# openai/gym

Measured on AMD Instinct MI355X. Metric: env-steps/sec at num_envs=2^20, CartPole-v1, higher is better.
Workload: dtype f64

## Files before the change

gym_amd/csrc/mxv_subnorm.hip:

```cpp
#include <hip/hip_runtime.h>

#include <cmath>
#include <cstdint>
#include <new>
#include <string>
#include <vector>

#include "../../include/mxv.h"
#include "mxv_divide.hpp"
#include "mxv_host.hpp"

using mxv::check_aligned;
using mxv::fail;
using mxv::last_error;

namespace {

constexpr int kThreads = 256;

template <int D>
__device__ __forceinline__ void load_row(const float *base, int64_t row, float (&v)[D]) {
    if constexpr (D == 4) {
        const float4 q = reinterpret_cast<const float4 *>(base)[row];
        v[0] = q.x; v[1] = q.y; v[2] = q.z; v[3] = q.w;
    } else if constexpr (D == 2) {
        const float2 q = reinterpret_cast<const float2 *>(base)[row];
        v[0] = q.x; v[1] = q.y;
    } else if constexpr (D == 6) {
        const float2 *p = reinterpret_cast<const float2 *>(base) + row * 3;
        const float2 a = p[0], b = p[1], c = p[2];
        v[0] = a.x; v[1] = a.y; v[2] = b.x; v[3] = b.y; v[4] = c.x; v[5] = c.y;
    } else {
#pragma unroll
        for (int j = 0; j < D; ++j) v[j] = base[row * D + j];
    }
}

template <int D>
__device__ __forceinline__ void store_row(float *base, int64_t row, const double (&y)[D]) {
    if constexpr (D == 4) {
        reinterpret_cast<float4 *>(base)[row] = make_float4((float)y[0], (float)y[1], (float)y[2], (float)y[3]);
    } else if constexpr (D == 2) {
        reinterpret_cast<float2 *>(base)[row] = make_float2((float)y[0], (float)y[1]);
    } else if constexpr (D == 6) {
        float2 *p = reinterpret_cast<float2 *>(base) + row * 3;
        p[0] = make_float2((float)y[0], (float)y[1]);
        p[1] = make_float2((float)y[2], (float)y[3]);
        p[2] = make_float2((float)y[4], (float)y[5]);
    } else {
#pragma unroll
        for (int j = 0; j < D; ++j) base[row * D + j] = (float)y[j];
    }
}

template <int D>
__device__ __forceinline__ void store_row(double *base, int64_t row, const double (&y)[D]) {
    if constexpr (D % 2 == 0) {
        double2 *p = reinterpret_cast<double2 *>(base) + row * (D / 2);
#pragma unroll
        for (int j = 0; j < D / 2; ++j) p[j] = make_double2(y[2 * j], y[2 * j + 1]);
    } else {
#pragma unroll
        for (int j = 0; j < D; ++j) base[row * D + j] = y[j];
    }
}

using mxv::div_shared;
using mxv::plain_delta;
using mxv::plain_divisor;
using mxv::plain_operand;
using mxv::refined_rcp;

template <int D>
__device__ __forceinline__ void update_one(const float (&x)[D], double (&mean)[D], double (&var)[D], double &count) {
    const double tot = count + 1.0;
    double delta[D], sq[D];
    bool ok = plain_divisor(tot) && (plain_divisor(count) || count == 0.0);
#pragma unroll
    for (int j = 0; j < D; ++j) {
        delta[j] = (double)x[j] - mean[j];
        sq[j] = (delta[j] * delta[j]) * count;
        ok = ok && plain_delta(delta[j]);
    }
    if (__all(ok)) {
        const double r = refined_rcp(tot);
        double m2[D];
        bool ok2 = true;
#pragma unroll
        for (int j = 0; j < D; ++j) {
            m2[j] = var[j] * count + div_shared(sq[j], tot, r);
            mean[j] = mean[j] + div_shared(delta[j], tot, r);
            ok2 = ok2 && plain_operand(m2[j]);
        }
        if (__all(ok2)) {
#pragma unroll
            for (int j = 0; j < D; ++j) var[j] = div_shared(m2[j], tot, r);
        } else {
#pragma unroll
            for (int j = 0; j < D; ++j) var[j] = m2[j] / tot;
        }
    } else {
#pragma unroll
        for (int j = 0; j < D; ++j) {
            const double m2 = var[j] * count + sq[j] / tot;
            mean[j] = mean[j] + delta[j] / tot;
            var[j] = m2 / tot;
        }
    }
    count = tot;
}

template <int D>
__device__ __forceinline__ void normalise(const float (&x)[D], const double (&mean)[D], const double (&var)[D], double eps, double (&y)[D]) {
#pragma unroll
    for (int j = 0; j < D; ++j) y[j] = ((double)x[j] - mean[j]) / sqrt(var[j] + eps);
}

struct SubObsArgs {
    const float *x;
    const float *fin;
    const uint8_t *te, *tr;
    void *y;
    double *yfin;
    double *stat;
    int64_t n;
    int32_t K;
    double eps;
};

template <int D, typename OUT>
__global__ void __launch_bounds__(kThreads) subnorm_obs_kernel(const SubObsArgs a) {
    const int64_t e = (int64_t)blockIdx.x * kThreads + threadIdx.x;
    const bool mine = e < a.n;
    const int64_t ec = mine ? e : 0;
    double mean[D], var[D], count;
#pragma unroll
    for (int j = 0; j < D; ++j) {
        mean[j] = a.stat[(int64_t)j * a.n + ec];
        var[j] = a.stat[(int64_t)(D + j) * a.n + ec];
    }
    count = a.stat[(int64_t)(2 * D) * a.n + ec];
    int kl = mine ? 0 : a.K;
    bool fin_done = false;
    const bool has_fin = a.te != nullptr && a.fin != nullptr;
    while (__any(kl < a.K)) {
        if (kl < a.K) {
            const int64_t r = (int64_t)kl * a.n + e;
            const bool use_fin = has_fin && !fin_done && ((a.te[r] | a.tr[r]) != 0);
            float x[D];
            load_row<D>(use_fin ? a.fin : a.x, r, x);
            double y[D];
            update_one<D>(x, mean, var, count);
            normalise<D>(x, mean, var, a.eps, y);
            if (use_fin) {
                if (a.yfin != nullptr) store_row<D>(a.yfin, r, y);
                fin_done = true;
            } else {
                store_row<D>(static_cast<OUT *>(a.y), r, y);
                fin_done = false;
                kl += 1;
            }
        }
    }
    if (!mine) return;
#pragma unroll
    for (int j = 0; j < D; ++j) {
        a.stat[(int64_t)j * a.n + e] = mean[j];
        a.stat[(int64_t)(D + j) * a.n + e] = var[j];
    }
    a.stat[(int64_t)(2 * D) * a.n + e] = count;
}

struct SubRewArgs {
    const void *rew;
    const uint8_t *te, *tr;
    void *out;
    double *stat;
    double *returns;
    int64_t n;
    int32_t K;
    double gamma, eps;
};

template <typename RT>
__global__ void __launch_bounds__(kThreads) subnorm_rew_kernel(const SubRewArgs a) {
    const int64_t e = (int64_t)blockIdx.x * kThreads + threadIdx.x;
    if (e >= a.n) return;
    double mean = a.stat[e], var = a.stat[a.n + e], count = a.stat[2 * a.n + e], ret = a.returns[e];
    const RT *rew = static_cast<const RT *>(a.rew);
    RT *out = static_cast<RT *>(a.out);
    for (int k = 0; k < a.K; ++k) {
        const int64_t r = (int64_t)k * a.n + e;
        const double rw = (double)rew[r];
        const bool done = (a.te[r] | a.tr[r]) != 0;
        ret = ret * a.gamma + rw;
        {
            const double tot = count + 1.0, delta = ret - mean, sq = (delta * delta) * count;
            const bool ok = plain_divisor(tot) && (plain_divisor(count) || count == 0.0) && plain_delta(delta);
            if (__all(ok)) {
                const double rc = refined_rcp(tot);
                const double m2 = var * count + div_shared(sq, tot, rc);
                mean = mean + div_shared(delta, tot, rc);
                var = __all(plain_operand(m2)) ? div_shared(m2, tot, rc) : m2 / tot;
            } else {
                const double m2 = var * count + sq / tot;
                mean = mean + delta / tot;
                var = m2 / tot;
            }
            count = tot;
        }
        out[r] = (RT)(rw / sqrt(var + a.eps));
        if (done) ret = 0.0;
    }
    a.stat[e] = mean;
    a.stat[a.n + e] = var;
    a.stat[2 * a.n + e] = count;
    a.returns[e] = ret;
}

}

struct mxv_subnorm {
    static constexpr const char *kNullMessage = "NULL mxv_subnorm";
    int device = 0, dim = 0;
    int64_t n = 0;
    hipStream_t stream = nullptr;
    double *stat = nullptr;
    double *returns = nullptr;
    std::string error;
};

namespace {

bool sub_dim_supported(int d) { return d == 1 || d == 2 || d == 3 || d == 4 || d == 6; }

int sub_checks(mxv_subnorm *nm, int32_t K) {
    MXV_CHECK(nm);
    if (K <= 0) return fail(nm, MXV_ERR_INVALID_ARG, "K must be positive (got %d)", K);
    if ((int64_t)K * nm->n > ((int64_t)1 << 40)) return fail(nm, MXV_ERR_INVALID_ARG, "K * num_envs too large");
    MXV_HIP(nm, hipSetDevice(nm->device));
    return MXV_OK;
}

int init_stats(mxv_subnorm *nm) {
    const size_t n = (size_t)nm->n;
    std::vector<double> init((size_t)(2 * nm->dim + 1) * n, 0.0);
    for (size_t i = (size_t)nm->dim * n; i < (size_t)(2 * nm->dim) * n; ++i) init[i] = 1.0;
    for (size_t i = (size_t)(2 * nm->dim) * n; i < init.size(); ++i) init[i] = 1e-4;
    MXV_HIP(nm, hipMemcpy(nm->stat, init.data(), init.size() * sizeof(double), hipMemcpyHostToDevice));
    MXV_HIP(nm, hipMemset(nm->returns, 0, n * sizeof(double)));
    return MXV_OK;
}

template <typename OUT>
int launch_obs(mxv_subnorm *nm, const SubObsArgs &a) {
    const dim3 grid((unsigned)((a.n + kThreads - 1) / kThreads)), block(kThreads);
    switch (nm->dim) {
        case 1: hipLaunchKernelGGL((subnorm_obs_kernel<1, OUT>), grid, block, 0, nm->stream, a); break;
        case 2: hipLaunchKernelGGL((subnorm_obs_kernel<2, OUT>), grid, block, 0, nm->stream, a); break;
        case 3: hipLaunchKernelGGL((subnorm_obs_kernel<3, OUT>), grid, block, 0, nm->stream, a); break;
        case 4: hipLaunchKernelGGL((subnorm_obs_kernel<4, OUT>), grid, block, 0, nm->stream, a); break;
        default: hipLaunchKernelGGL((subnorm_obs_kernel<6, OUT>), grid, block, 0, nm->stream, a); break;
    }
    MXV_HIP(nm, hipGetLastError());
    return MXV_OK;
}

}

extern "C" {

int mxv_subnorm_create(int32_t device, int32_t dim, int64_t num_envs, void *stream, mxv_subnorm **out) {
    if (!out) return fail<mxv_subnorm>(nullptr, MXV_ERR_INVALID_ARG, "NULL output pointer");
    *out = nullptr;
    if (!sub_dim_supported(dim)) return fail<mxv_subnorm>(nullptr, MXV_ERR_UNSUPPORTED, "dim must be one of 1, 2, 3, 4, 6 (got %d)", dim);
    if (num_envs <= 0 || num_envs > ((int64_t)1 << 31)) return fail<mxv_subnorm>(nullptr, MXV_ERR_INVALID_ARG, "num_envs must be in 1 .. 2^31");
    int ndev = 0;
    hipError_t e = hipGetDeviceCount(&ndev);
    if (e != hipSuccess || ndev <= 0)
        return fail<mxv_subnorm>(nullptr, MXV_ERR_HIP, "no HIP device available (%s): the engine has no CPU fallback",
                     e != hipSuccess ? hipGetErrorString(e) : "device count 0");
    if (device < 0 || device >= ndev) return fail<mxv_subnorm>(nullptr, MXV_ERR_INVALID_ARG, "device %d out of range", device);
    mxv_subnorm *nm = new (std::nothrow) mxv_subnorm();
    if (!nm) return fail<mxv_subnorm>(nullptr, MXV_ERR_INVALID_ARG, "out of host memory");
    nm->device = device;
    nm->dim = dim;
    nm->n = num_envs;
    nm->stream = (hipStream_t)stream;
    hipError_t err = hipSetDevice(device);
    if (err == hipSuccess) err = hipMalloc((void **)&nm->stat, (size_t)(2 * dim + 1) * (size_t)num_envs * sizeof(double));
    if (err == hipSuccess) err = hipMalloc((void **)&nm->returns, (size_t)num_envs * sizeof(double));
    if (err != hipSuccess || init_stats(nm) != MXV_OK) {
        fail<mxv_subnorm>(nullptr, MXV_ERR_HIP, "mxv_subnorm_create: %s", err != hipSuccess ? hipGetErrorString(err) : nm->error.c_str());
        mxv_subnorm_destroy(nm);
        return MXV_ERR_HIP;
    }
    *out = nm;
    return MXV_OK;
}

int mxv_subnorm_destroy(mxv_subnorm *nm) {
    if (!nm) return MXV_OK;
    (void)hipSetDevice(nm->device);
    (void)hipStreamSynchronize(nm->stream);
    if (nm->stat) (void)hipFree(nm->stat);
    if (nm->returns) (void)hipFree(nm->returns);
    delete nm;
    return MXV_OK;
}

const char *mxv_subnorm_last_error(const mxv_subnorm *nm) { return last_error(nm); }

int mxv_subnorm_set_stream(mxv_subnorm *nm, void *stream) {
    MXV_CHECK(nm);
    MXV_HIP(nm, hipSetDevice(nm->device));
    MXV_HIP(nm, hipStreamSynchronize(nm->stream));
    nm->stream = (hipStream_t)stream;
    return MXV_OK;
}

int mxv_subnorm_get_state(mxv_subnorm *nm, double *mean_host, double *var_host, double *count_host, double *returns_host) {
    MXV_CHECK(nm);
    MXV_HIP(nm, hipSetDevice(nm->device));
    const size_t n = (size_t)nm->n, D = (size_t)nm->dim;
    std::vector<double> st((2 * D + 1) * n);
    MXV_HIP(nm, hipMemcpyAsync(st.data(), nm->stat, st.size() * sizeof(double), hipMemcpyDeviceToHost, nm->stream));
    if (returns_host) MXV_HIP(nm, hipMemcpyAsync(returns_host, nm->returns, n * sizeof(double), hipMemcpyDeviceToHost, nm->stream));
    MXV_HIP(nm, hipStreamSynchronize(nm->stream));
    for (size_t i = 0; i < n; ++i) {
        for (size_t j = 0; j < D; ++j) {
            if (mean_host) mean_host[i * D + j] = st[j * n + i];
            if (var_host) var_host[i * D + j] = st[(D + j) * n + i];
        }
        if (count_host) count_host[i] = st[2 * D * n + i];
    }
    return MXV_OK;
}

int mxv_subnorm_set_state(mxv_subnorm *nm, const double *mean_host, const double *var_host, const double *count_host,
                          const double *returns_host) {
    MXV_CHECK(nm);
    if (!mean_host || !var_host || !count_host) return fail(nm, MXV_ERR_INVALID_ARG, "mean / var / count pointer is NULL");
    MXV_HIP(nm, hipSetDevice(nm->device));
    const size_t n = (size_t)nm->n, D = (size_t)nm->dim;
    std::vector<double> st((2 * D + 1) * n);
    for (size_t i = 0; i < n; ++i) {
        for (size_t j = 0; j < D; ++j) {
            st[j * n + i] = mean_host[i * D + j];
            st[(D + j) * n + i] = var_host[i * D + j];
        }
        st[2 * D * n + i] = count_host[i];
    }
    MXV_HIP(nm, hipMemcpyAsync(nm->stat, st.data(), st.size() * sizeof(double), hipMemcpyHostToDevice, nm->stream));
    if (returns_host) MXV_HIP(nm, hipMemcpyAsync(nm->returns, returns_host, n * sizeof(double), hipMemcpyHostToDevice, nm->stream));
    MXV_HIP(nm, hipStreamSynchronize(nm->stream));
    return MXV_OK;
}

int mxv_subnorm_observations(mxv_subnorm *nm, int32_t K, const float *x_dev, const float *final_dev, const uint8_t *terminated_dev,
                             const uint8_t *truncated_dev, void *y_dev, int32_t out_f32, double *final_y_dev, double epsilon) {
    if (int rc = sub_checks(nm, K)) return rc;
    if (!x_dev || !y_dev) return fail(nm, MXV_ERR_INVALID_ARG, "x / y pointer is NULL");
    if ((terminated_dev == nullptr) != (truncated_dev == nullptr))
        return fail(nm, MXV_ERR_INVALID_ARG, "terminated and truncated go together (both NULL: nobody has finished, the reset() form)");
    if (final_dev && !terminated_dev) return fail(nm, MXV_ERR_INVALID_ARG, "terminal observations without the flags that say whose they are");
    if (final_y_dev && !final_dev) return fail(nm, MXV_ERR_INVALID_ARG, "final_y without the terminal observations");
    if (!out_f32 && (const void *)x_dev == (const void *)y_dev)
        return fail(nm, MXV_ERR_INVALID_ARG, "float64 results cannot alias the float32 observations");
    {
        const int D = nm->dim;
        const size_t a32 = D % 4 == 0 ? 16 : (D % 2 == 0 ? 8 : 4), a64 = D % 2 == 0 ? 16 : 8;
        const struct { const void *p; size_t b; const char *what; } t[] = {{x_dev, a32, "x"}, {final_dev, a32, "final"}, {y_dev, out_f32 ? a32 : a64, "y"},
                                                                           {final_y_dev, a64, "final_y"}};
        for (const auto &e : t)
            if (int rc = check_aligned(nm, e.p, e.b, e.what)) return rc;
    }
    SubObsArgs a{x_dev, final_dev, terminated_dev, truncated_dev, y_dev, final_y_dev, nm->stat, nm->n, K, epsilon};
    return out_f32 ? launch_obs<float>(nm, a) : launch_obs<double>(nm, a);
}

int mxv_subnorm_rewards(mxv_subnorm *nm, int32_t K, const void *reward_dev, int32_t reward_f32, const uint8_t *terminated_dev,
                        const uint8_t *truncated_dev, void *out_dev, double gamma, double epsilon) {
    if (int rc = sub_checks(nm, K)) return rc;
    if (nm->dim != 1) return fail(nm, MXV_ERR_INVALID_ARG, "reward statistics need dim == 1 (got %d)", nm->dim);
    if (!reward_dev || !terminated_dev || !truncated_dev || !out_dev) return fail(nm, MXV_ERR_INVALID_ARG, "NULL device pointer");
    if ((((uintptr_t)reward_dev | (uintptr_t)out_dev) & (reward_f32 ? 3u : 7u)) != 0)
        return fail(nm, MXV_ERR_INVALID_ARG, "reward / out pointer is not %d-byte aligned", reward_f32 ? 4 : 8);
    SubRewArgs a{reward_dev, terminated_dev, truncated_dev, out_dev, nm->stat, nm->returns, nm->n, K, gamma, epsilon};
    const dim3 grid((unsigned)((a.n + kThreads - 1) / kThreads)), block(kThreads);
    if (reward_f32)
        hipLaunchKernelGGL(subnorm_rew_kernel<float>, grid, block, 0, nm->stream, a);
    else
        hipLaunchKernelGGL(subnorm_rew_kernel<double>, grid, block, 0, nm->stream, a);
    MXV_HIP(nm, hipGetLastError());
    return MXV_OK;
}

}
```

Baseline: 184.7 billion.

## Prefetch next rows, use guarded rsqrt for f32 output, defer final-obs stores

Restructures the observation normalisation kernel so the next step's row and the done flags two steps ahead are loaded before the current step is computed, hiding load latency. For f32 outputs it replaces the f64 divide-by-sqrt with a refined hardware rsqrt, guarded against inputs out of range and rounding near a midpoint, and falls back to the exact path when any lane is unsafe. Final-observation rows for done envs are queued per wavefront in shared memory and normalised and stored in batches, which reduces divergence. The cost is more code complexity and extra shared-memory use, which may lower occupancy.

```diff
diff --git a/gym_amd/csrc/mxv_rsqrt.hpp b/gym_amd/csrc/mxv_rsqrt.hpp
--- /dev/null
+++ b/gym_amd/csrc/mxv_rsqrt.hpp
@@ -0,0 +1,30 @@
+#pragma once
+#include <hip/hip_runtime.h>
+#include <stdint.h>
+
+namespace mxv {
+
+__device__ __forceinline__ bool rsqrt_guard(double v) { return ((uint32_t)__double2hiint(v) >> 20) - 959u < 129u; }
+
+__device__ __forceinline__ double rsqrt_refined(double v) {
+    const double r0 = __builtin_amdgcn_rsq(v);
+    const double e = __fma_rn(-(v * r0), r0, 1.0);
+    return __fma_rn(r0 * e, __fma_rn(0.375, e, 0.5), r0);
+}
+
+constexpr uint32_t kF32Band = 512;
+
+__device__ __forceinline__ bool f32_round_unsafe(double y) {
+    const uint32_t lo = (uint32_t)__double2loint(y), hi = (uint32_t)__double2hiint(y);
+    const bool near_mid = ((lo - ((1u << 28) - kF32Band)) & 0x1fffffffu) <= 2 * kF32Band;
+    const bool in_range = ((hi >> 20) & 0x7ffu) - 897u < 253u;
+    return near_mid || !in_range;
+}
+
+__device__ __forceinline__ double f32_quotient(double d, double v, bool &unsafe) {
+    const double y = d * rsqrt_refined(v);
+    unsafe = !rsqrt_guard(v) || f32_round_unsafe(y);
+    return y;
+}
+
+}
diff --git a/gym_amd/csrc/mxv_subnorm.hip b/gym_amd/csrc/mxv_subnorm.hip
--- a/gym_amd/csrc/mxv_subnorm.hip
+++ b/gym_amd/csrc/mxv_subnorm.hip
@@ -9,6 +9,7 @@
 #include "../../include/mxv.h"
 #include "mxv_divide.hpp"
 #include "mxv_host.hpp"
+#include "mxv_rsqrt.hpp"
 
 using mxv::check_aligned;
 using mxv::fail;
@@ -54,6 +55,23 @@
 }
 
 template <int D>
+__device__ __forceinline__ void store_row(float *base, int64_t row, const float (&y)[D]) {
+    if constexpr (D == 4) {
+        reinterpret_cast<float4 *>(base)[row] = make_float4(y[0], y[1], y[2], y[3]);
+    } else if constexpr (D == 2) {
+        reinterpret_cast<float2 *>(base)[row] = make_float2(y[0], y[1]);
+    } else if constexpr (D == 6) {
+        float2 *p = reinterpret_cast<float2 *>(base) + row * 3;
+        p[0] = make_float2(y[0], y[1]);
+        p[1] = make_float2(y[2], y[3]);
+        p[2] = make_float2(y[4], y[5]);
+    } else {
+#pragma unroll
+        for (int j = 0; j < D; ++j) base[row * D + j] = y[j];
+    }
+}
+
+template <int D>
 __device__ __forceinline__ void store_row(double *base, int64_t row, const double (&y)[D]) {
     if constexpr (D % 2 == 0) {
         double2 *p = reinterpret_cast<double2 *>(base) + row * (D / 2);
@@ -111,9 +129,61 @@
 }
 
 template <int D>
-__device__ __forceinline__ void normalise(const float (&x)[D], const double (&mean)[D], const double (&var)[D], double eps, double (&y)[D]) {
-#pragma unroll
-    for (int j = 0; j < D; ++j) y[j] = ((double)x[j] - mean[j]) / sqrt(var[j] + eps);
+__device__ __forceinline__ void normalise_operands(const float (&x)[D], const double (&mean)[D], const double (&var)[D], double eps,
+                                                   double (&d)[D], double (&v)[D]) {
+#pragma unroll
+    for (int j = 0; j < D; ++j) {
+        d[j] = (double)x[j] - mean[j];
+        v[j] = var[j] + eps;
+    }
+}
+template <int D>
+__device__ __forceinline__ void normalise_exact(const double (&d)[D], const double (&v)[D], double (&y)[D]) {
+#pragma unroll
+    for (int j = 0; j < D; ++j) y[j] = d[j] / sqrt(v[j]);
+}
+
+using mxv::f32_quotient;
+
+template <int D>
+__device__ __forceinline__ void normalise_f32(const double (&d)[D], const double (&v)[D], double (&y)[D]) {
+    bool unsafe = false;
+#pragma unroll
+    for (int j = 0; j < D; ++j) {
+        bool u;
+        y[j] = f32_quotient(d[j], v[j], u);
+        unsafe = unsafe || u;
+    }
+    if (__any(unsafe)) normalise_exact<D>(d, v, y);
+}
+
+constexpr int kQueue = 64;
+constexpr int kWaves = kThreads / 64;
+
+template <int D>
+struct FinQueue {
+    double dv[kWaves][2 * D][kQueue];
+    int64_t row[kWaves][kQueue];
+};
+
+template <int D>
+__device__ __forceinline__ void flush_queue(FinQueue<D> &q, int w, int lane, int pending, double *yfin) {
+    __builtin_amdgcn_fence(__ATOMIC_RELEASE, "wavefront");
+    __builtin_amdgcn_wave_barrier();
+    __builtin_amdgcn_fence(__ATOMIC_ACQUIRE, "wavefront");
+    if (lane < pending) {
+        double d[D], v[D], y[D];
+#pragma unroll
+        for (int j = 0; j < D; ++j) {
+            d[j] = q.dv[w][j][lane];
+            v[j] = q.dv[w][D + j][lane];
+        }
+        normalise_exact<D>(d, v, y);
+        store_row<D>(yfin, q.row[w][lane], y);
+    }
+    __builtin_amdgcn_fence(__ATOMIC_RELEASE, "wavefront");
+    __builtin_amdgcn_wave_barrier();
+    __builtin_amdgcn_fence(__ATOMIC_ACQUIRE, "wavefront");
 }
 
 struct SubObsArgs {
@@ -141,27 +211,87 @@
     }
     count = a.stat[(int64_t)(2 * D) * a.n + ec];
     int kl = mine ? 0 : a.K;
-    bool fin_done = false;
     const bool has_fin = a.te != nullptr && a.fin != nullptr;
+    __shared__ FinQueue<D> queue;
+    const int w = threadIdx.x >> 6, lane = threadIdx.x & 63;
+    int pending = 0;
+    bool cur_fin = false;
+    bool next_done = false;
+    float x[D];
+    const int klast = a.K - 1;
+    if (mine) {
+        if (has_fin) {
+            cur_fin = (a.te[e] | a.tr[e]) != 0;
+            if (klast >= 1) next_done = (a.te[a.n + e] | a.tr[a.n + e]) != 0;
+        }
+        load_row<D>(cur_fin ? a.fin : a.x, e, x);
+    }
+    __builtin_amdgcn_s_waitcnt(0x0f70);
     while (__any(kl < a.K)) {
+        bool push = false;
+        double d[D], v[D];
+        int64_t r = 0;
         if (kl < a.K) {
-            const int64_t r = (int64_t)kl * a.n + e;
-            const bool use_fin = has_fin && !fin_done && ((a.te[r] | a.tr[r]) != 0);
-            float x[D];
-            load_row<D>(use_fin ? a.fin : a.x, r, x);
-            double y[D];
+            r = (int64_t)kl * a.n + e;
+            const bool next_fin = !cur_fin && next_done;
+            const int kn = cur_fin ? kl : kl + 1;
+            float xn[D] = {};
+            if (kn <= klast) load_row<D>(next_fin ? a.fin : a.x, (int64_t)kn * a.n + e, xn);
+            uint8_t te2 = 0, tr2 = 0;
+            if (has_fin && !cur_fin && kl + 2 <= klast) {
+                const int64_t r2 = (int64_t)(kl + 2) * a.n + e;
+                te2 = a.te[r2];
+                tr2 = a.tr[r2];
+            }
             update_one<D>(x, mean, var, count);
-            normalise<D>(x, mean, var, a.eps, y);
-            if (use_fin) {
-                if (a.yfin != nullptr) store_row<D>(a.yfin, r, y);
-                fin_done = true;
+            normalise_operands<D>(x, mean, var, a.eps, d, v);
+            const bool batch = !cur_fin;
+            OUT y[D] = {};
+            if (batch) {
+                double y64[D];
+                if constexpr (sizeof(OUT) == sizeof(float))
+                    normalise_f32<D>(d, v, y64);
+                else
+                    normalise_exact<D>(d, v, y64);
+#pragma unroll
+                for (int j = 0; j < D; ++j) y[j] = (OUT)y64[j];
+            }
+#pragma unroll
+            for (int j = 0; j < D; ++j) {
+                x[j] = xn[j];
+                asm volatile("" : "+v"(x[j]) : : "memory");
+            }
+            const bool done2 = (te2 | tr2) != 0;
+            if (batch) {
+                store_row<D>(static_cast<OUT *>(a.y), r, y);
+                kl += 1;
+                cur_fin = next_fin;
+                next_done = done2;
             } else {
-                store_row<D>(static_cast<OUT *>(a.y), r, y);
-                fin_done = false;
-                kl += 1;
-            }
-        }
-    }
+                push = a.yfin != nullptr;
+                cur_fin = false;
+            }
+        }
+        const unsigned long long pushing = __ballot(push);
+        if (pushing != 0) {
+            const int np = __popcll(pushing);
+            if (pending + np > kQueue) {
+                flush_queue<D>(queue, w, lane, pending, a.yfin);
+                pending = 0;
+            }
+            if (push) {
+                const int slot = pending + (int)__builtin_amdgcn_mbcnt_hi((uint32_t)(pushing >> 32), __builtin_amdgcn_mbcnt_lo((uint32_t)pushing, 0u));
+#pragma unroll
+                for (int j = 0; j < D; ++j) {
+                    queue.dv[w][j][slot] = d[j];
+                    queue.dv[w][D + j][slot] = v[j];
+                }
+                queue.row[w][slot] = r;
+            }
+            pending += np;
+        }
+    }
+    if (pending != 0) flush_queue<D>(queue, w, lane, pending, a.yfin);
     if (!mine) return;
 #pragma unroll
     for (int j = 0; j < D; ++j) {
```

Result: no change. 184.5 billion (-0.1%).
